# ChengZhang-98/lqer

Hardware: AMD Instinct MI355X
Metric: W4A8+rank-r Linear GEMM TFLOPS-equiv (higher is better)
Workload: dtype bf16; 1 GPU; LqerLinear 4096x4096 rank32 W4A8-MXINT16 M=2048 (BASELINE configs[1]); rank=32, formats=x MXINT8/16, W MXINT4/16, A_out,B_out as x, y fp16, weights=one Linear

## Files before the change

### lqer_amd/csrc/act16_fused.hip

```cpp
#include "common.h"

namespace lqer {
namespace a16f {

constexpr int ROWS = 8, WAVES = 8, SLAB = 512, PITCH = 1040;

__host__ inline size_t lds_bytes(int rp) { return (size_t)WAVES * ROWS * PITCH + (size_t)WAVES * ROWS * rp * sizeof(float); }

typedef __attribute__((ext_vector_type(8))) __bf16 bf16v8;

#ifdef LQER_CLOCKPROBE
__device__ unsigned long long* g_a16_stamp_buf = nullptr;
#define A16_STAMP(i) asm volatile("s_memtime %0\n\ts_waitcnt lgkmcnt(0)" : "=s"(cp[i])::"memory")
#else
#define A16_STAMP(i)
#endif

template <int DT, int RT>
__global__ __launch_bounds__(512) void k_act16_fused(const void* __restrict__ x, int64_t M, int64_t K, int64_t ld, QP qx, bf16_t* __restrict__ xq,
                                                      int64_t Kp, const bf16_t* __restrict__ a_frag, QP qa, int L_aout, bf16_t* __restrict__ xaq) {
  constexpr int RP = 16 * RT;
  constexpr int HB = RT == 8 ? 2 : (RT == 4 ? 4 : 8);
  constexpr int NPART = 16 / HB;
  extern __shared__ __attribute__((aligned(16))) unsigned char smem[];
  const int lane = threadIdx.x & 63;
  const int wave = __builtin_amdgcn_readfirstlane(threadIdx.x >> 6);
  unsigned char* const wb = smem + (size_t)wave * ROWS * PITCH;
  float* const red = (float*)(smem + (size_t)WAVES * ROWS * PITCH);
  const int64_t m0 = (int64_t)blockIdx.x * ROWS;
  const int nslab = (int)((Kp + SLAB - 1) / SLAB);
  const int g = lane >> 4;
  const unsigned char* const tok = wb + (lane & 7) * PITCH + 16 * g;
  const u32x4* const fr = (const u32x4*)a_frag + lane;
  f32x4 acc[RT];
#pragma unroll
  for (int t = 0; t < RT; ++t) acc[t] = (f32x4){0.f, 0.f, 0.f, 0.f};
#ifdef LQER_CLOCKPROBE
  unsigned long long cp[8] = {0, 0, 0, 0, 0, 0, 0, 0};
  A16_STAMP(0);
#endif

  for (int s = wave; s < nslab; s += WAVES) {
    const int64_t k0 = (int64_t)s * SLAB + 8 * lane;
    const bool in_img = k0 < Kp, in_x = k0 < K;
    u32x4 raw[ROWS];
#pragma unroll
    for (int r = 0; r < ROWS; ++r)
      raw[r] = (in_x && m0 + r < M) ? *(const u32x4*)((const bf16_t*)x + (m0 + r) * ld + k0) : (u32x4){0, 0, 0, 0};
    const int st0 = s * (SLAB / 32), nst = (int)(Kp / 32);
    u32x4 fa[HB][RT], fb[HB][RT];
    auto load_part = [&](u32x4 (&f)[HB][RT], int part) {
#pragma unroll
      for (int i = 0; i < HB; ++i)
#pragma unroll
        for (int t = 0; t < RT; ++t) {
          const int st = st0 + part * HB + i;
          f[i][t] = fr[((int64_t)(st < nst ? st : 0) * RT + t) * 64];
        }
    };
    if (s == wave) A16_STAMP(1);
#pragma unroll
    for (int r = 0; r < ROWS; ++r) {
      if (r == 1 && s == wave) A16_STAMP(2);
      if (r == 2) {
        asm volatile("" ::: "memory");
        load_part(fa, 0);
        asm volatile("" ::: "memory");
      }
      if (r == 5) {
        asm volatile("" ::: "memory");
        load_part(fb, 1);
        asm volatile("" ::: "memory");
      }
      float v[8];
      const uint32_t wd[4] = {raw[r][0], raw[r][1], raw[r][2], raw[r][3]};
#pragma unroll
      for (int j = 0; j < 4; ++j) {
        if constexpr (DT == LQER_F16) {
          typedef __attribute__((ext_vector_type(2))) _Float16 h2;
          const h2 h = __builtin_bit_cast(h2, wd[j]);
          v[2 * j] = (float)h[0], v[2 * j + 1] = (float)h[1];
        } else {
          v[2 * j] = __uint_as_float(wd[j] << 16), v[2 * j + 1] = __uint_as_float(wd[j] & 0xffff0000u);
        }
      }
      float amax = 0.f;
#pragma unroll
      for (int i = 0; i < 8; ++i) amax = fmaxf(amax, fabsf(v[i]));
      amax = fmaxf(amax, __shfl_xor(amax, 1, 64));
      uint32_t w[4] = {0, 0, 0, 0};
      if (amax > 0.f) {
        const int e = block_exponent_u(amax, qx);
        if (mxint16_fast_ok(e, qx)) {
          mxint16_bf16_fast<DT != LQER_F16, 8>(v, e, qx, w);
        } else {
#pragma unroll
          for (int i = 0; i < 4; ++i) {
            const uint32_t lo = exact_bf16_bits(ldexpf(mxint_mantissa(v[2 * i], e, qx), e - qx.mbits));
            const uint32_t hi = exact_bf16_bits(ldexpf(mxint_mantissa(v[2 * i + 1], e, qx), e - qx.mbits));
            w[i] = lo | (hi << 16);
          }
        }
      }
      const u32x4 wv = {w[0], w[1], w[2], w[3]};
      if (in_img) *(u32x4*)(xq + (m0 + r) * Kp + k0) = wv;
      *(u32x4*)(wb + r * PITCH + 16 * lane) = wv;
    }
    if (s == wave) A16_STAMP(3);
    __builtin_amdgcn_fence(__ATOMIC_RELEASE, "wavefront");
    __builtin_amdgcn_wave_barrier();
    __builtin_amdgcn_fence(__ATOMIC_ACQUIRE, "wavefront");
    auto half = [&](const u32x4 (&f)[HB][RT], int t0) {
      u32x4 tk[HB];
#pragma unroll
      for (int i = 0; i < HB; ++i) tk[i] = *(const u32x4*)(tok + 64 * (t0 + i));
#pragma unroll
      for (int i = 0; i < HB; ++i)
#pragma unroll
        for (int t = 0; t < RT; ++t)
          acc[t] = __builtin_amdgcn_mfma_f32_16x16x32_bf16(__builtin_bit_cast(bf16v8, tk[i]), __builtin_bit_cast(bf16v8, f[i][t]), acc[t], 0, 0, 0);
    };
#pragma unroll
    for (int pp = 0; pp < NPART; pp += 2) {
      half(fa, pp * HB);
      if (pp + 2 < NPART) load_part(fa, pp + 2);
      half(fb, (pp + 1) * HB);
      if (pp + 3 < NPART) load_part(fb, pp + 3);
    }
    __builtin_amdgcn_fence(__ATOMIC_RELEASE, "wavefront");
    __builtin_amdgcn_wave_barrier();
#ifdef LQER_CLOCKPROBE
    if (s == wave) {
      asm volatile("" ::"v"(acc[0]));
      A16_STAMP(4);
    }
#endif
  }
  if (g < 2) {
#pragma unroll
    for (int t = 0; t < RT; ++t)
#pragma unroll
      for (int j = 0; j < 4; ++j) red[(wave * ROWS + 4 * g + j) * RP + 16 * t + (lane & 15)] = acc[t][j];
  }
  __syncthreads();
#ifdef LQER_CLOCKPROBE
  A16_STAMP(5);
  if (g_a16_stamp_buf && lane == 0) {
    unsigned long long* o = g_a16_stamp_buf + ((size_t)blockIdx.x * WAVES + wave) * 8;
    for (int i = 1; i < 6; ++i) o[i] = cp[i] - cp[0];
    unsigned long long rt;
    asm volatile("s_memrealtime %0\n\ts_waitcnt lgkmcnt(0)" : "=s"(rt)::"memory");
    o[0] = cp[0], o[6] = rt;
  }
#endif
  const int tid = threadIdx.x;
  const bool live = tid < ROWS * RP / 4;
  const int r = tid / (RP / 4), c4 = tid - r * (RP / 4);
  float4 sum = make_float4(0.f, 0.f, 0.f, 0.f);
  if (live) {
#pragma unroll
    for (int w = 0; w < WAVES; ++w) {
      const float4 v = *(const float4*)(red + (w * ROWS + r) * RP + 4 * c4);
      sum.x += v.x, sum.y += v.y, sum.z += v.z, sum.w += v.w;
    }
  }
  if (tid >= 64 * ((ROWS * RP / 4 + 63) / 64)) return;
  float bmax = fmaxf(fmaxf(fabsf(sum.x), fabsf(sum.y)), fmaxf(fabsf(sum.z), fabsf(sum.w)));
  const int G = L_aout / 4;
  for (int d = 1; d < G; d <<= 1) bmax = fmaxf(bmax, __shfl_xor(bmax, d, 64));
  if (!live || m0 + r >= M) return;
  const bool anyb = bmax > 0.f;
  const int eb = anyb ? block_exponent(bmax, qa) : 0;
  const float v[4] = {sum.x, sum.y, sum.z, sum.w};
  uint32_t w2[2];
#pragma unroll
  for (int i = 0; i < 2; ++i) {
    const float m0v = anyb ? mxint_mantissa(v[2 * i], eb, qa) : 0.f;
    const float m1v = anyb ? mxint_mantissa(v[2 * i + 1], eb, qa) : 0.f;
    w2[i] = exact_bf16_bits(ldexpf(m0v, eb - qa.mbits)) | (exact_bf16_bits(ldexpf(m1v, eb - qa.mbits)) << 16);
  }
  *(uint2*)(xaq + ((m0 + r) * RP + 4 * c4)) = make_uint2(w2[0], w2[1]);
}

__global__ __launch_bounds__(256) void k_a_b16(const bf16_t* __restrict__ limb0, int64_t Kp, int rp, bf16_t* __restrict__ out) {
  const int RT = rp / 16;
  const int64_t n_img = (int64_t)rp * Kp / 8, total = 2 * n_img;
  for (int64_t idx = (int64_t)blockIdx.x * 256 + threadIdx.x; idx < total; idx += (int64_t)gridDim.x * 256) {
    if (idx < n_img) {
      ((u32x4*)out)[idx] = ((const u32x4*)limb0)[idx];
    } else {
      const int64_t f = idx - n_img;
      const int lane = (int)(f & 63);
      const int64_t blk = f >> 6;
      const int t = (int)(blk % RT);
      const int64_t s = blk / RT;
      ((u32x4*)out)[idx] = *(const u32x4*)(limb0 + (int64_t)(16 * t + (lane & 15)) * Kp + 32 * s + 8 * (lane >> 4));
    }
  }
}

}

#ifdef LQER_CLOCKPROBE
extern "C" int lqer_debug_set_a16_stamp_buffer(void* p) { return (int)hipMemcpyToSymbol(HIP_SYMBOL(a16f::g_a16_stamp_buf), &p, sizeof(p)); }
#endif

size_t a_b16_image_bytes(int64_t K, int64_t r) { return (size_t)2 * lqer_padded_r(r) * lqer_padded_k(K) * sizeof(bf16_t); }

int a_b16_prepare_dispatch(const void* a_t_limbs, int64_t K, int64_t r, void* out, hipStream_t st) {
  const int64_t rp = lqer_padded_r(r), Kp = lqer_padded_k(K);
  if (rp % 16 != 0 || Kp % 32 != 0) {
    set_error("a_b16_prepare: padded rank %d / padded K %d", (int)rp, (int)Kp);
    return LQER_E_UNSUPPORTED;
  }
  const int64_t total = 2 * rp * Kp / 8;
  a16f::k_a_b16<<<(unsigned)((total + 255) / 256 < 4096 ? (total + 255) / 256 : 4096), 256, 0, st>>>((const bf16_t*)a_t_limbs, Kp, (int)rp, (bf16_t*)out);
  return check_launch("a_b16_prepare");
}

int act16_fused_dispatch(const void* x, int dtype, int64_t M, int64_t K, int64_t ldx, const QP& qx, bf16_t* xq, const void* a_b16, int64_t r,
                         const QP& qa, bf16_t* xaq, int tuning, hipStream_t st) {
  if (tuning & LQER_TUNE_ACT16_SPLIT) return LQER_E_UNSUPPORTED;
  const int64_t rp = lqer_padded_r(r), Kp = lqer_padded_k(K);
  if (dtype == LQER_F32 || !a_b16 || !xaq || !xq || r <= 0 || M <= 0) return LQER_E_UNSUPPORTED;
  if (!(rp == 16 || rp == 32 || rp == 64)) return LQER_E_UNSUPPORTED;
  if (qx.kind != LQER_Q_MXINT || qx.block != 16 || qx.mbits > 8) return LQER_E_UNSUPPORTED;
  if (((uintptr_t)x % 16) != 0 || ((ldx * 2) % 16) != 0 || K % 16 != 0) return LQER_E_UNSUPPORTED;
  if (qa.kind != LQER_Q_MXINT || qa.mbits > 8) return LQER_E_UNSUPPORTED;
  const int L = (qa.block <= 0 || qa.block >= rp) ? (int)rp : qa.block;
  const int G = L / 4;
  if (rp % L != 0 || L % 4 != 0 || (G & (G - 1)) != 0 || G > 64) return LQER_E_UNSUPPORTED;
  if (!(tuning & LQER_TUNE_ACT16_FUSED) && (M > LQER_ACT8_FUSED_MAX_M || M < LQER_ACT8_FUSED_MIN_M)) return LQER_E_UNSUPPORTED;
  const bf16_t* const a_frag = (const bf16_t*)a_b16 + rp * Kp;
  const unsigned grid = (unsigned)((M + a16f::ROWS - 1) / a16f::ROWS);
  const int lds = (int)a16f::lds_bytes((int)rp);
  auto run = [&](auto dt) {
    constexpr int DT = decltype(dt)::value, LIMIT = 160 * 1024;
    const char* const what = "quantize_act_xa (fused block-16 route)";
    switch (rp / 16) {
      case 1: return launch_k<a16f::k_act16_fused<DT, 1>, LIMIT>(what, grid, 512, lds, st, x, M, K, ldx, qx, xq, Kp, a_frag, qa, L, xaq);
      case 2: return launch_k<a16f::k_act16_fused<DT, 2>, LIMIT>(what, grid, 512, lds, st, x, M, K, ldx, qx, xq, Kp, a_frag, qa, L, xaq);
      default: return launch_k<a16f::k_act16_fused<DT, 4>, LIMIT>(what, grid, 512, lds, st, x, M, K, ldx, qx, xq, Kp, a_frag, qa, L, xaq);
    }
  };
  return dtype == LQER_F16 ? run(std::integral_constant<int, LQER_F16>{}) : run(std::integral_constant<int, LQER_BF16>{});
}

}
```

Measured before the change: 1050 TFLOP/s-equiv.

## Use buffer loads/stores and branchless fast quantize with deferred slow-path fixup

Result: no change. 1060 TFLOP/s-equiv, median of 6 (+0.9%).

```diff
diff --git a/lqer_amd/csrc/act16_fused.hip b/lqer_amd/csrc/act16_fused.hip
--- a/lqer_amd/csrc/act16_fused.hip
+++ b/lqer_amd/csrc/act16_fused.hip
@@ -16,12 +16,42 @@
 #define A16_STAMP(i)
 #endif
 
+__device__ __forceinline__ int block_exponent_h16(float amax, const QP& q) {
+  const int e = (int)((__float_as_uint(amax) + 0x7fffffu) >> 23) - 127;
+  return e < q.emin ? q.emin : (e > q.emax ? q.emax : e);
+}
+
+template <int DT>
+__device__ __forceinline__ void unpack8(u32x4 raw, float (&v)[8]) {
+  const uint32_t wd[4] = {raw[0], raw[1], raw[2], raw[3]};
+#pragma unroll
+  for (int j = 0; j < 4; ++j) {
+    if constexpr (DT == LQER_F16) {
+      typedef __attribute__((ext_vector_type(2))) _Float16 h2;
+      const h2 h = __builtin_bit_cast(h2, wd[j]);
+      v[2 * j] = (float)h[0], v[2 * j + 1] = (float)h[1];
+    } else {
+      v[2 * j] = __uint_as_float(wd[j] << 16), v[2 * j + 1] = __uint_as_float(wd[j] & 0xffff0000u);
+    }
+  }
+}
+
+__device__ __forceinline__ float block16_amax(const float (&v)[8]) {
+  float amax = 0.f;
+#pragma unroll
+  for (int i = 0; i < 8; ++i) amax = fmaxf(amax, fabsf(v[i]));
+  return fmaxf(amax, __int_as_float(__builtin_amdgcn_update_dpp(0, __float_as_int(amax), 0xB1, 0xf, 0xf, true)));
+}
+
 template <int DT, int RT>
 __global__ __launch_bounds__(512) void k_act16_fused(const void* __restrict__ x, int64_t M, int64_t K, int64_t ld, QP qx, bf16_t* __restrict__ xq,
                                                       int64_t Kp, const bf16_t* __restrict__ a_frag, QP qa, int L_aout, bf16_t* __restrict__ xaq) {
+  static_assert(DT == LQER_F16 || DT == LQER_BF16, "block_exponent_h16 needs a 16-bit input type");
   constexpr int RP = 16 * RT;
   constexpr int HB = RT == 8 ? 2 : (RT == 4 ? 4 : 8);
   constexpr int NPART = 16 / HB;
+  asm volatile("" ::"s"(x), "s"(M), "s"(K), "s"(ld), "s"(xq), "s"(Kp), "s"(a_frag), "s"(xaq), "s"(L_aout), "s"(qx.mbits), "s"(qx.emin), "s"(qx.emax),
+               "s"(qx.mmax), "s"(qx.mneg), "s"(qx.eps), "s"(qx.tiny), "s"(qa.mbits), "s"(qa.emin), "s"(qa.emax), "s"(qa.mmax), "s"(qa.mneg), "s"(qa.eps), "s"(qa.tiny));
   extern __shared__ __attribute__((aligned(16))) unsigned char smem[];
   const int lane = threadIdx.x & 63;
   const int wave = __builtin_amdgcn_readfirstlane(threadIdx.x >> 6);
@@ -32,6 +62,11 @@
   const int g = lane >> 4;
   const unsigned char* const tok = wb + (lane & 7) * PITCH + 16 * g;
   const u32x4* const fr = (const u32x4*)a_frag + lane;
+  const int ldb = (int)(2 * ld), kpb = (int)(2 * Kp);
+  const int nrows = (int)(M - m0 < ROWS ? M - m0 : ROWS);
+  const int x_bytes = (nrows - 1) * ldb + (int)(2 * K), q_bytes = ROWS * kpb;
+  const auto x_rsrc = __builtin_amdgcn_make_buffer_rsrc((void*)((const bf16_t*)x + m0 * ld), 0, x_bytes, 0x00020000);
+  const auto q_rsrc = __builtin_amdgcn_make_buffer_rsrc((void*)(xq + m0 * Kp), 0, q_bytes, 0x00020000);
   f32x4 acc[RT];
 #pragma unroll
   for (int t = 0; t < RT; ++t) acc[t] = (f32x4){0.f, 0.f, 0.f, 0.f};
@@ -42,11 +77,11 @@
 
   for (int s = wave; s < nslab; s += WAVES) {
     const int64_t k0 = (int64_t)s * SLAB + 8 * lane;
-    const bool in_img = k0 < Kp, in_x = k0 < K;
+    const int xoff = k0 < K ? (int)(2 * k0) : x_bytes;
+    const int qoff = k0 < Kp ? (int)(2 * k0) : q_bytes;
     u32x4 raw[ROWS];
 #pragma unroll
-    for (int r = 0; r < ROWS; ++r)
-      raw[r] = (in_x && m0 + r < M) ? *(const u32x4*)((const bf16_t*)x + (m0 + r) * ld + k0) : (u32x4){0, 0, 0, 0};
+    for (int r = 0; r < ROWS; ++r) raw[r] = __builtin_bit_cast(u32x4, __builtin_amdgcn_raw_buffer_load_b128(x_rsrc, xoff + r * ldb, 0, 0));
     const int st0 = s * (SLAB / 32), nst = (int)(Kp / 32);
     u32x4 fa[HB][RT], fb[HB][RT];
     auto load_part = [&](u32x4 (&f)[HB][RT], int part) {
@@ -58,10 +93,19 @@
           f[i][t] = fr[((int64_t)(st < nst ? st : 0) * RT + t) * 64];
         }
     };
-    if (s == wave) A16_STAMP(1);
+#ifdef LQER_CLOCKPROBE
+    if (s == wave) {
+      A16_STAMP(1);
+      asm volatile("s_waitcnt vmcnt(7)" : "+v"(raw[0])::"memory");
+      A16_STAMP(7);
+    }
+#endif
+    bool slow = false;
 #pragma unroll
     for (int r = 0; r < ROWS; ++r) {
+#ifdef LQER_CLOCKPROBE
       if (r == 1 && s == wave) A16_STAMP(2);
+#endif
       if (r == 2) {
         asm volatile("" ::: "memory");
         load_part(fa, 0);
@@ -73,40 +117,42 @@
         asm volatile("" ::: "memory");
       }
       float v[8];
-      const uint32_t wd[4] = {raw[r][0], raw[r][1], raw[r][2], raw[r][3]};
-#pragma unroll
-      for (int j = 0; j < 4; ++j) {
-        if constexpr (DT == LQER_F16) {
-          typedef __attribute__((ext_vector_type(2))) _Float16 h2;
-          const h2 h = __builtin_bit_cast(h2, wd[j]);
-          v[2 * j] = (float)h[0], v[2 * j + 1] = (float)h[1];
-        } else {
-          v[2 * j] = __uint_as_float(wd[j] << 16), v[2 * j + 1] = __uint_as_float(wd[j] & 0xffff0000u);
-        }
-      }
-      float amax = 0.f;
-#pragma unroll
-      for (int i = 0; i < 8; ++i) amax = fmaxf(amax, fabsf(v[i]));
-      amax = fmaxf(amax, __shfl_xor(amax, 1, 64));
-      uint32_t w[4] = {0, 0, 0, 0};
-      if (amax > 0.f) {
-        const int e = block_exponent_u(amax, qx);
-        if (mxint16_fast_ok(e, qx)) {
-          mxint16_bf16_fast<DT != LQER_F16, 8>(v, e, qx, w);
-        } else {
+      unpack8<DT>(raw[r], v);
+      const float amax = block16_amax(v);
+      const int e = block_exponent_h16(amax, qx);
+      const bool any = amax > 0.f;
+      slow |= any && !mxint16_fast_ok(e, qx);
+      uint32_t w[4];
+      mxint16_bf16_fast<DT != LQER_F16, 8>(v, e, qx, w);
+      const u32x4 wv = {any ? w[0] : 0u, any ? w[1] : 0u, any ? w[2] : 0u, any ? w[3] : 0u};
+      __builtin_amdgcn_raw_buffer_store_b128(wv, q_rsrc, qoff + r * kpb, 0, 0);
+      *(u32x4*)(wb + r * PITCH + 16 * lane) = wv;
+    }
+    if (__builtin_amdgcn_ballot_w64(slow) != 0) {
+      asm volatile("s_waitcnt vmcnt(0)" ::: "memory");
+#pragma unroll 1
+      for (int r = 0; r < ROWS; ++r) {
+        const u32x4 rw = __builtin_bit_cast(u32x4, __builtin_amdgcn_raw_buffer_load_b128(x_rsrc, xoff + r * ldb, 0, 0));
+        float v[8];
+        unpack8<DT>(rw, v);
+        const float amax = block16_amax(v);
+        const int e = block_exponent_h16(amax, qx);
+        if (amax > 0.f && !mxint16_fast_ok(e, qx)) {
+          u32x4 wv;
 #pragma unroll
           for (int i = 0; i < 4; ++i) {
             const uint32_t lo = exact_bf16_bits(ldexpf(mxint_mantissa(v[2 * i], e, qx), e - qx.mbits));
             const uint32_t hi = exact_bf16_bits(ldexpf(mxint_mantissa(v[2 * i + 1], e, qx), e - qx.mbits));
-            w[i] = lo | (hi << 16);
+            wv[i] = lo | (hi << 16);
           }
+          __builtin_amdgcn_raw_buffer_store_b128(wv, q_rsrc, qoff + r * kpb, 0, 0);
+          *(u32x4*)(wb + r * PITCH + 16 * lane) = wv;
         }
       }
-      const u32x4 wv = {w[0], w[1], w[2], w[3]};
-      if (in_img) *(u32x4*)(xq + (m0 + r) * Kp + k0) = wv;
-      *(u32x4*)(wb + r * PITCH + 16 * lane) = wv;
-    }
+    }
+#ifdef LQER_CLOCKPROBE
     if (s == wave) A16_STAMP(3);
+#endif
     __builtin_amdgcn_fence(__ATOMIC_RELEASE, "wavefront");
     __builtin_amdgcn_wave_barrier();
     __builtin_amdgcn_fence(__ATOMIC_ACQUIRE, "wavefront");
@@ -148,6 +194,7 @@
   if (g_a16_stamp_buf && lane == 0) {
     unsigned long long* o = g_a16_stamp_buf + ((size_t)blockIdx.x * WAVES + wave) * 8;
     for (int i = 1; i < 6; ++i) o[i] = cp[i] - cp[0];
+    o[7] = cp[7] - cp[0];
     unsigned long long rt;
     asm volatile("s_memrealtime %0\n\ts_waitcnt lgkmcnt(0)" : "=s"(rt)::"memory");
     o[0] = cp[0], o[6] = rt;
@@ -226,6 +273,7 @@
   if (!(rp == 16 || rp == 32 || rp == 64)) return LQER_E_UNSUPPORTED;
   if (qx.kind != LQER_Q_MXINT || qx.block != 16 || qx.mbits > 8) return LQER_E_UNSUPPORTED;
   if (((uintptr_t)x % 16) != 0 || ((ldx * 2) % 16) != 0 || K % 16 != 0) return LQER_E_UNSUPPORTED;
+  if (ldx < K || ldx > (INT32_MAX >> 5) || Kp > (INT32_MAX >> 5)) return LQER_E_UNSUPPORTED;
   if (qa.kind != LQER_Q_MXINT || qa.mbits > 8) return LQER_E_UNSUPPORTED;
   const int L = (qa.block <= 0 || qa.block >= rp) ? (int)rp : qa.block;
   const int G = L / 4;
```
